# ru1ven/KeypointFusion

Measured on AMD Instinct MI355X. Metric: RGB-D img/sec fwd (B=64, 256x256), higher is better.
Workload: dtype f32; 1 GPU; KPFusion-convnext-tiny, depth+RGB UNet backbones forward, B=64/GPU 256x256 f32 (BASELINE configs[1]); batch_per_gpu=64, global_batch=64, input=256x256, parallelism=dp1 (batch shards, no collective)

## Files before the change

### keypointfusion_amd/csrc/kpf_mlp.hip

```cpp
#include "kpf_common.h"
#include <stdlib.h>
#include <type_traits>

namespace {

typedef __attribute__((address_space(3))) void lds_void_t;
typedef __attribute__((address_space(1))) void gbl_void_t;

__device__ __attribute__((aligned(16))) float kpf_mlp_zero16[4] = {0.f, 0.f, 0.f, 0.f};

struct MlpArgs {
  const float* y;
  const float* x;
  const float* w1;
  const float* b1;
  const float* w2;
  const float* b2;
  const float* gamma;
  float* out;
  const float* zero;
  int M;
};

__device__ __forceinline__ float gelu_f(float x) {
  const float z = fabsf(x) * 0.70710678118654752440f;
  const float t = __builtin_amdgcn_rcpf(fmaf(0.3275911f, z, 1.0f));
  float p = fmaf(1.061405429f, t, -1.453152027f);
  p = fmaf(p, t, 1.421413741f);
  p = fmaf(p, t, -0.284496736f);
  p = fmaf(p, t, 0.254829592f);
  const float e = __builtin_amdgcn_exp2f(-1.4426950408889634f * z * z);
  const float q = 0.5f * x * (p * t) * e;
  return fmaxf(x, 0.f) - fabsf(q);
}

template <int RC>
__device__ __forceinline__ int row_sw(int r) {
  static_assert(RC % 8 == 0, "row length must be a multiple of 32 floats");
  return (RC % 16 == 0) ? (r & 15) : ((r >> 1) & 7);
}

template <int ROWS, int RC, int NT>
__device__ __forceinline__ void dma_image(float* lds_dst, const float* src, long src_ld, int valid_rows, const float* zero, int tid) {
  static_assert((ROWS * RC) % NT == 0, "image must be a whole number of workgroup-wide passes");
  constexpr int PASSES = ROWS * RC / NT;
  const int wave = tid >> 6;
#pragma unroll
  for (int p = 0; p < PASSES; ++p) {
    const int pos = p * NT + tid;
    const int r = pos / RC, cp = pos - r * RC;
    const int c = cp ^ row_sw<RC>(r);
    const float* s = r < valid_rows ? src + (long)r * src_ld + 4 * c : zero;
    __builtin_amdgcn_global_load_lds((gbl_void_t*)s, (lds_void_t*)(lds_dst + (p * NT + wave * 64) * 4), 16, 0, 0);
  }
}

template <int NC, int TM, int HT, int NW>
__global__ __launch_bounds__(64 * NW) void convnext_mlp_kernel(const MlpArgs a) {
  constexpr int NT = 64 * NW;
  constexpr int C = 16 * NC;
  constexpr int H4 = 4 * C;
  constexpr int HC = 16 * HT;
  constexpr int BM = 16 * TM * NW;
  constexpr int RCY = C / 4;
  constexpr int RCW = HC / 4;
  constexpr int NCH = H4 / HC;
  constexpr int YF = BM * C, W1F = HC * C, W2F = C * HC;
  static_assert(H4 % HC == 0, "chunking");

  extern __shared__ __attribute__((aligned(16))) float lds[];
  float* Ys = lds;
  float* W1s = Ys + YF;
  float* W2s = W1s + 2 * W1F;
  float* B1s = W2s + 2 * W2F;

  const int tid = threadIdx.x, lane = tid & 63, wave = tid >> 6;
  const int fr = lane & 15, fg = lane >> 4;
  const long m0 = (long)blockIdx.x * BM;
  const int valid = (int)((a.M - m0) < BM ? (a.M - m0) : BM);

  dma_image<BM, RCY, NT>(Ys, a.y + m0 * C, C, valid, a.zero, tid);
  dma_image<HC, RCY, NT>(W1s, a.w1, C, HC, a.zero, tid);
  dma_image<C, RCW, NT>(W2s, a.w2, H4, C, a.zero, tid);

  const f32x4 zero4 = {0.f, 0.f, 0.f, 0.f};
  f32x4 acc2[NC][TM];
#pragma unroll
  for (int n = 0; n < NC; ++n)
#pragma unroll
    for (int j = 0; j < TM; ++j) acc2[n][j] = zero4;

  float* B2s = B1s + H4;
  float* Gs = B2s + C;
  for (int i = tid; i < H4; i += NT) B1s[i] = a.b1[i];
  for (int i = tid; i < C; i += NT) {
    B2s[i] = a.b2[i];
    Gs[i] = a.gamma[i];
  }
  __syncthreads();

  const int yrow0 = wave * TM * 16 + fr;
  for (int ch = 0; ch < NCH; ++ch) {
    const int cur = ch & 1;
    if (ch + 1 < NCH) {
      dma_image<HC, RCY, NT>(W1s + (cur ^ 1) * W1F, a.w1 + (long)(ch + 1) * HC * C, C, HC, a.zero, tid);
      dma_image<C, RCW, NT>(W2s + (cur ^ 1) * W2F, a.w2 + (long)(ch + 1) * HC, H4, C, a.zero, tid);
    }
    const float* w1b = W1s + cur * W1F;
    const float* w2b = W2s + cur * W2F;

    f32x4 acc1[HT][TM];
#pragma unroll
    for (int h = 0; h < HT; ++h)
#pragma unroll
      for (int j = 0; j < TM; ++j) acc1[h][j] = zero4;
#pragma unroll
    for (int s = 0; s < NC; ++s) {
      f32x4 yf[TM], wf[HT];
#pragma unroll
      for (int j = 0; j < TM; ++j) {
        const int r = yrow0 + j * 16;
        yf[j] = *reinterpret_cast<const f32x4*>(Ys + r * C + (((4 * s + fg) ^ row_sw<RCY>(r)) << 2));
      }
#pragma unroll
      for (int h = 0; h < HT; ++h) {
        const int r = h * 16 + fr;
        wf[h] = *reinterpret_cast<const f32x4*>(w1b + r * C + (((4 * s + fg) ^ row_sw<RCY>(r)) << 2));
      }
#pragma unroll
      for (int e = 0; e < 4; ++e)
#pragma unroll
        for (int h = 0; h < HT; ++h)
#pragma unroll
          for (int j = 0; j < TM; ++j) acc1[h][j] = __builtin_amdgcn_mfma_f32_16x16x4f32(wf[h][e], yf[j][e], acc1[h][j], 0, 0, 0);
    }

#pragma unroll
    for (int h = 0; h < HT; ++h) {
      const f32x4 bv = *reinterpret_cast<const f32x4*>(B1s + ch * HC + h * 16 + 4 * fg);
#pragma unroll
      for (int j = 0; j < TM; ++j)
#pragma unroll
        for (int e = 0; e < 4; ++e) acc1[h][j][e] = gelu_f(acc1[h][j][e] + bv[e]);
      f32x4 wf[NC];
#pragma unroll
      for (int n = 0; n < NC; ++n) {
        const int r = n * 16 + fr;
        wf[n] = *reinterpret_cast<const f32x4*>(w2b + r * HC + (((4 * h + fg) ^ row_sw<RCW>(r)) << 2));
      }
#pragma unroll
      for (int e = 0; e < 4; ++e)
#pragma unroll
        for (int n = 0; n < NC; ++n)
#pragma unroll
          for (int j = 0; j < TM; ++j) acc2[n][j] = __builtin_amdgcn_mfma_f32_16x16x4f32(wf[n][e], acc1[h][j][e], acc2[n][j], 0, 0, 0);
    }
    __syncthreads();
  }

#pragma unroll
  for (int j = 0; j < TM; ++j) {
    const long m = m0 + wave * TM * 16 + j * 16 + fr;
    if (m >= a.M) continue;
    f32x4 xv[NC];
#pragma unroll
    for (int n = 0; n < NC; ++n) xv[n] = *reinterpret_cast<const f32x4*>(a.x + m * C + n * 16 + 4 * fg);
#pragma unroll
    for (int n = 0; n < NC; ++n) {
      const int c = n * 16 + 4 * fg;
      const f32x4 bv = *reinterpret_cast<const f32x4*>(B2s + c);
      const f32x4 gv = *reinterpret_cast<const f32x4*>(Gs + c);
      f32x4 v;
#pragma unroll
      for (int e = 0; e < 4; ++e) v[e] = xv[n][e] + gv[e] * (acc2[n][j][e] + bv[e]);
      *reinterpret_cast<f32x4*>(a.out + m * C + c) = v;
    }
  }
}

struct MlpSplitArgs {
  const float* y;
  const float* x;
  const float* w1;
  const float* b1;
  const float* w2;
  const float* b2;
  const float* gamma;
  float* out;
  const float* zero;
  float us1, us2;
  int M;
};

template <int NC, int HT, int NW, bool YLDS, int TM>
__global__ __launch_bounds__(64 * NW) void convnext_mlp_split_kernel(const MlpSplitArgs a) {
  constexpr int NT = 64 * NW;
  constexpr int C = 16 * NC;
  constexpr int KC = C / 32;
  constexpr int H4 = 4 * C;
  constexpr int HC = 16 * HT;
  constexpr int HK = HC / 32;
  constexpr int BM = 16 * TM * NW;
  constexpr int RCY = C / 4, RCW = HC / 4;
  constexpr int NCH = H4 / HC;
  constexpr int YF = YLDS ? BM * C : 0, W1F = HC * C, W2F = C * HC;
  static_assert(C % 32 == 0 && HC % 32 == 0 && H4 % HC == 0, "split blocks are 32 wide");

  extern __shared__ __attribute__((aligned(16))) float lds[];
  float* Ys = lds;
  float* W1s = Ys + YF;
  float* W2s = W1s + 2 * W1F;
  float* B1s = W2s + 2 * W2F;
  float* B2s = B1s + H4;
  float* Gs = B2s + C;

  const int tid = threadIdx.x, lane = tid & 63, wave = tid >> 6;
  const int fr = lane & 15, fg = lane >> 4;
  const long m0 = (long)blockIdx.x * BM;
  const int valid = (int)((a.M - m0) < BM ? (a.M - m0) : BM);

  if (YLDS) dma_image<BM, RCY, NT>(Ys, a.y + m0 * C, C, valid, a.zero, tid);
  dma_image<HC, RCY, NT>(W1s, a.w1, C, HC, a.zero, tid);
  dma_image<C, RCW, NT>(W2s, a.w2, H4, C, a.zero, tid);

  const f32x4 zero4 = {0.f, 0.f, 0.f, 0.f};
  f32x4 acc2[NC][TM];
#pragma unroll
  for (int n = 0; n < NC; ++n)
#pragma unroll
    for (int j = 0; j < TM; ++j) acc2[n][j] = zero4;
  for (int i = tid; i < H4; i += NT) B1s[i] = a.b1[i];
  for (int i = tid; i < C; i += NT) {
    B2s[i] = a.b2[i];
    Gs[i] = a.gamma[i];
  }
  __syncthreads();

  f16x8 yh[KC][TM], yl[KC][TM];
#pragma unroll
  for (int j = 0; j < TM; ++j) {
    const int yr = (wave * TM + j) * 16 + fr;
    if (YLDS) {
#pragma unroll
      for (int k = 0; k < KC; ++k) {
        yh[k][j] = *reinterpret_cast<const f16x8*>(Ys + yr * C + (((8 * k + fg) ^ row_sw<RCY>(yr)) << 2));
        yl[k][j] = *reinterpret_cast<const f16x8*>(Ys + yr * C + (((8 * k + 4 + fg) ^ row_sw<RCY>(yr)) << 2));
      }
    } else {
      const long mr = (m0 + yr < a.M) ? m0 + yr : a.M - 1;
      const float* yrow = a.y + mr * C;
#pragma unroll
      for (int k = 0; k < KC; ++k) {
        yh[k][j] = *reinterpret_cast<const f16x8*>(yrow + ((8 * k + fg) << 2));
        yl[k][j] = *reinterpret_cast<const f16x8*>(yrow + ((8 * k + 4 + fg) << 2));
      }
    }
  }
  const float us1 = a.us1;

  for (int ch = 0; ch < NCH; ++ch) {
    const int cur = ch & 1;
    if (ch + 1 < NCH) {
      dma_image<HC, RCY, NT>(W1s + (cur ^ 1) * W1F, a.w1 + (long)(ch + 1) * HC * C, C, HC, a.zero, tid);
      dma_image<C, RCW, NT>(W2s + (cur ^ 1) * W2F, a.w2 + (long)(ch + 1) * HC, H4, C, a.zero, tid);
    }
    const float* w1b = W1s + cur * W1F;
    const float* w2b = W2s + cur * W2F;

    f32x4 acc1[HT][TM];
#pragma unroll
    for (int h = 0; h < HT; ++h)
#pragma unroll
      for (int j = 0; j < TM; ++j) acc1[h][j] = zero4;
#pragma unroll
    for (int k = 0; k < KC; ++k) {
#pragma unroll
      for (int h = 0; h < HT; ++h) {
        const int r = h * 16 + fr;
        const f16x8 wh = *reinterpret_cast<const f16x8*>(w1b + r * C + (((8 * k + fg) ^ row_sw<RCY>(r)) << 2));
        const f16x8 wl = *reinterpret_cast<const f16x8*>(w1b + r * C + (((8 * k + 4 + fg) ^ row_sw<RCY>(r)) << 2));
#pragma unroll
        for (int j = 0; j < TM; ++j) {
          acc1[h][j] = __builtin_amdgcn_mfma_f32_16x16x32_f16(wl, yh[k][j], acc1[h][j], 0, 0, 0);
          acc1[h][j] = __builtin_amdgcn_mfma_f32_16x16x32_f16(wh, yl[k][j], acc1[h][j], 0, 0, 0);
          acc1[h][j] = __builtin_amdgcn_mfma_f32_16x16x32_f16(wh, yh[k][j], acc1[h][j], 0, 0, 0);
        }
      }
    }

#pragma unroll
    for (int q = 0; q < HK; ++q) {
      f16x8 hh[TM], hl[TM];
#pragma unroll
      for (int t = 0; t < 2; ++t) {
        const int h = 2 * q + t;
        const f32x4 bv = *reinterpret_cast<const f32x4*>(B1s + ch * HC + h * 16 + 4 * fg);
#pragma unroll
        for (int j = 0; j < TM; ++j)
#pragma unroll
          for (int e = 0; e < 4; ++e) {
            const float g = gelu_f(fmaf(acc1[h][j][e], us1, bv[e]));
            const _Float16 hi = (_Float16)g;
            hh[j][4 * t + e] = hi;
            hl[j][4 * t + e] = (_Float16)(g - (float)hi);
          }
      }
#pragma unroll
      for (int n = 0; n < NC; ++n) {
        const int r = n * 16 + fr;
        const f16x8 wh = *reinterpret_cast<const f16x8*>(w2b + r * HC + (((8 * q + fg) ^ row_sw<RCW>(r)) << 2));
        const f16x8 wl = *reinterpret_cast<const f16x8*>(w2b + r * HC + (((8 * q + 4 + fg) ^ row_sw<RCW>(r)) << 2));
#pragma unroll
        for (int j = 0; j < TM; ++j) {
          acc2[n][j] = __builtin_amdgcn_mfma_f32_16x16x32_f16(wl, hh[j], acc2[n][j], 0, 0, 0);
          acc2[n][j] = __builtin_amdgcn_mfma_f32_16x16x32_f16(wh, hl[j], acc2[n][j], 0, 0, 0);
          acc2[n][j] = __builtin_amdgcn_mfma_f32_16x16x32_f16(wh, hh[j], acc2[n][j], 0, 0, 0);
        }
      }
    }
    __syncthreads();
  }

  const float us2 = a.us2;
#pragma unroll
  for (int j = 0; j < TM; ++j) {
    const long m = m0 + (wave * TM + j) * 16 + fr;
    if (m >= a.M) continue;
    f32x4 xv[NC];
#pragma unroll
    for (int n = 0; n < NC; ++n) xv[n] = *reinterpret_cast<const f32x4*>(a.x + m * C + n * 16 + 4 * fg);
#pragma unroll
    for (int n = 0; n < NC; ++n) {
      const int c = n * 16 + 4 * fg;
      const f32x4 bv = *reinterpret_cast<const f32x4*>(B2s + c);
      const f32x4 gv = *reinterpret_cast<const f32x4*>(Gs + c);
      f32x4 v;
#pragma unroll
      for (int e = 0; e < 4; ++e) v[e] = xv[n][e] + gv[e] * fmaf(acc2[n][j][e], us2, bv[e]);
      *reinterpret_cast<f32x4*>(a.out + m * C + c) = v;
    }
  }
}

struct Mlp16Args {
  const void* y;
  const void* x;
  const void* w1;
  const float* b1;
  const void* w2c;
  const float* b2;
  const float* gamma;
  void* out;
  int M;
  int dbg;
};

__device__ __forceinline__ float gelu_h16m(float x) { return kpf_gelu_h16(x); }

template <int C, int PT, int R, bool BF, int WPS = 2, int NW = 4>
__global__ __launch_bounds__(64 * NW, WPS) void convnext_mlp_h16_kernel(const Mlp16Args a) {
  using TH = typename std::conditional<BF, bf16_t, f16_t>::type;
  constexpr int NT = 64 * NW;
  constexpr int KC = C / 32;
  constexpr int NCT = C / 16;
  constexpr int NCH = 4 * C / 32;
  constexpr int W1B = 32 * C * 2;
  constexpr int W2B = C * 64;
  constexpr int CHB = W1B + W2B;
  constexpr int G = CHB / (NT * 16);
  constexpr int RC1 = C / 8;
  constexpr int BM = 16 * PT * NW;
  static_assert(C % 128 == 0 && R >= 2 && R <= 4 && W1B % (NT * 16) == 0 && W2B % (NT * 16) == 0, "shape");

  extern __shared__ __attribute__((aligned(16))) float lds[];
  char* const LB = reinterpret_cast<char*>(lds);
  constexpr int RING_B = R * CHB > NW * PT * 16 * 2 * C ? R * CHB : NW * PT * 16 * 2 * C;
  float* const B1s = reinterpret_cast<float*>(LB + RING_B);
  float* const B2s = B1s + 4 * C;
  float* const Gs = B2s + C;
  const int tid = threadIdx.x, lane = tid & 63;
  const int wave = __builtin_amdgcn_readfirstlane(tid >> 6);
  const int fr = lane & 15, fg = lane >> 4;
  const long m0 = (long)blockIdx.x * BM;

  f16x8 yf[KC][PT];
#pragma unroll
  for (int pt = 0; pt < PT; ++pt) {
    long m = m0 + (wave * PT + pt) * 16 + fr;
    m = m < a.M ? m : a.M - 1;
    const TH* yrow = reinterpret_cast<const TH*>(a.y) + m * C + 8 * fg;
#pragma unroll
    for (int ks = 0; ks < KC; ++ks) yf[ks][pt] = *reinterpret_cast<const f16x8*>(yrow + 32 * ks);
  }
  for (int i = tid; i < 4 * C; i += NT) B1s[i] = a.b1[i];
  for (int i = tid; i < C; i += NT) {
    B2s[i] = a.b2[i];
    Gs[i] = a.gamma[i];
  }
  __syncthreads();
  asm volatile("s_waitcnt vmcnt(0)" ::: "memory");

  const TH* const w1g = reinterpret_cast<const TH*>(a.w1);
  const TH* const w2g = reinterpret_cast<const TH*>(a.w2c);
  constexpr int P1 = W1B / (NT * 16), P2 = W2B / (NT * 16), RPP1 = NT / RC1;
  const int r1 = tid / RC1, cp1 = tid % RC1;
  const int s1a = r1 * C + 8 * (cp1 ^ (r1 & 15)), s1b = r1 * C + 8 * (cp1 ^ ((r1 + RPP1) & 15));
  const int s2 = (tid >> 2) * 32 + 8 * ((tid & 3) ^ ((tid >> 4) & 3));
  auto stage = [&](int ch, int slot) {
    char* dst = LB + slot * CHB + wave * 1024;
    const TH* const g1 = w1g + (long)ch * 32 * C;
    const TH* const g2 = w2g + (long)ch * C * 32;
#pragma unroll
    for (int p = 0; p < P1; ++p)
      __builtin_amdgcn_global_load_lds((gbl_void_t*)(g1 + ((p & 1) ? s1b : s1a) + p * RPP1 * C), (lds_void_t*)(dst + p * NT * 16), 16, 0, 0);
#pragma unroll
    for (int p = 0; p < P2; ++p)
      __builtin_amdgcn_global_load_lds((gbl_void_t*)(g2 + s2 + p * (NT / 4) * 32), (lds_void_t*)(dst + W1B + p * NT * 16), 16, 0, 0);
  };
  if (!(a.dbg & 4))
#pragma unroll
    for (int c = 0; c < R - 1; ++c) stage(c, c);

  f32x4 acc[NCT][PT];
#pragma unroll
  for (int n = 0; n < NCT; ++n)
#pragma unroll
    for (int pt = 0; pt < PT; ++pt) acc[n][pt] = f32x4{0.f, 0.f, 0.f, 0.f};
  const int w1_rd = fr * (2 * C), w2_rd = W1B + fr * 64 + ((fg ^ ((fr >> 2) & 3)) << 4);

  auto chunk = [&](int ch, auto SLOT) {
    constexpr int slot = decltype(SLOT)::value;
    const int younger = NCH - 1 - ch;
    if (a.dbg & 4) {
    } else if (younger >= R - 2) asm volatile("s_waitcnt vmcnt(%0)" ::"n"((R - 2) * G) : "memory");
    else if (R > 3 && younger == 1) asm volatile("s_waitcnt vmcnt(%0)" ::"n"(G) : "memory");
    else asm volatile("s_waitcnt vmcnt(0)" ::: "memory");
    __builtin_amdgcn_s_barrier();
    if (ch + R - 1 < NCH && !(a.dbg & 4)) stage(ch + R - 1, (slot + R - 1) % R);
    const char* const sb = LB + slot * CHB;
    f32x4 d1[2][PT];
#pragma unroll
    for (int ht = 0; ht < 2; ++ht)
#pragma unroll
      for (int pt = 0; pt < PT; ++pt) d1[ht][pt] = f32x4{0.f, 0.f, 0.f, 0.f};
#pragma unroll
    for (int ks = 0; ks < KC; ++ks)
#pragma unroll
      for (int ht = 0; ht < 2; ++ht) {
        const f16x8 w = *reinterpret_cast<const f16x8*>(sb + w1_rd + ht * 16 * (2 * C) + ((((4 * ks + fg) ^ fr) & (RC1 - 1)) << 4));
#pragma unroll
        for (int pt = 0; pt < PT; ++pt) {
          if constexpr (BF) d1[ht][pt] = __builtin_amdgcn_mfma_f32_16x16x32_bf16(__builtin_bit_cast(bf16x8, w), __builtin_bit_cast(bf16x8, yf[ks][pt]), d1[ht][pt], 0, 0, 0);
          else d1[ht][pt] = __builtin_amdgcn_mfma_f32_16x16x32_f16(w, yf[ks][pt], d1[ht][pt], 0, 0, 0);
        }
      }
    const f32x4 bv0 = *reinterpret_cast<const f32x4*>(B1s + ch * 32 + 4 * fg);
    const f32x4 bv1 = *reinterpret_cast<const f32x4*>(B1s + ch * 32 + 16 + 4 * fg);
    f16x8 hf[PT];
#pragma unroll
    for (int pt = 0; pt < PT; ++pt) {
      typename std::conditional<BF, bf16x8, f16x8>::type h;
#pragma unroll
      for (int e = 0; e < 4; ++e) {
        h[e] = (TH)((a.dbg & 1) ? d1[0][pt][e] + bv0[e] : gelu_h16m(d1[0][pt][e] + bv0[e]));
        h[4 + e] = (TH)((a.dbg & 1) ? d1[1][pt][e] + bv1[e] : gelu_h16m(d1[1][pt][e] + bv1[e]));
      }
      hf[pt] = __builtin_bit_cast(f16x8, h);
    }
#pragma unroll
    for (int n = 0; n < NCT; ++n) {
      const f16x8 w = *reinterpret_cast<const f16x8*>(sb + w2_rd + n * 16 * 64);
#pragma unroll
      for (int pt = 0; pt < PT; ++pt) {
        if constexpr (BF) acc[n][pt] = __builtin_amdgcn_mfma_f32_16x16x32_bf16(__builtin_bit_cast(bf16x8, w), __builtin_bit_cast(bf16x8, hf[pt]), acc[n][pt], 0, 0, 0);
        else acc[n][pt] = __builtin_amdgcn_mfma_f32_16x16x32_f16(w, hf[pt], acc[n][pt], 0, 0, 0);
      }
    }
  };
  static_assert(NCH % R == 0, "whole ring revolutions");
  for (int cb = 0; cb < NCH; cb += R) {
    chunk(cb, std::integral_constant<int, 0>{});
    chunk(cb + 1, std::integral_constant<int, 1 % R>{});
    if constexpr (R > 2) chunk(cb + 2, std::integral_constant<int, 2 % R>{});
    if constexpr (R > 3) chunk(cb + 3, std::integral_constant<int, 3 % R>{});
  }
  __builtin_amdgcn_s_barrier();

  const TH* const xg = reinterpret_cast<const TH*>(a.x);
  TH* const og = reinterpret_cast<TH*>(a.out);
  constexpr int ROWB = 2 * C;
  char* const stg = LB + wave * (PT * 16 * ROWB);
#pragma unroll
  for (int pt = 0; pt < PT; ++pt) {
    const long m = m0 + (wave * PT + pt) * 16 + fr;
    const long mr = m < a.M ? m : a.M - 1;
    f32x4 xv[NCT];
#pragma unroll
    for (int n = 0; n < NCT; ++n) xv[n] = kpf_ld4(xg + mr * C + n * 16 + 4 * fg);
#pragma unroll
    for (int n = 0; n < NCT; ++n) {
      const f32x4 bv = *reinterpret_cast<const f32x4*>(B2s + n * 16 + 4 * fg);
      const f32x4 gv = *reinterpret_cast<const f32x4*>(Gs + n * 16 + 4 * fg);
      f32x4 v;
#pragma unroll
      for (int e = 0; e < 4; ++e) v[e] = xv[n][e] + gv[e] * (acc[n][pt][e] + bv[e]);
      const int row = pt * 16 + fr, cidx = 2 * n + (fg >> 1);
      kpf_st4(reinterpret_cast<TH*>(stg + row * ROWB + ((cidx ^ fr) << 4) + (fg & 1) * 8), v);
    }
  }
  asm volatile("s_waitcnt lgkmcnt(0)" ::: "memory");
  constexpr int CPR = ROWB / 16, RPI = 64 / CPR;
  const int rl = lane / CPR, p = lane % CPR;
#pragma unroll
  for (int it = 0; it < PT * 16 / RPI; ++it) {
    const int row = it * RPI + rl;
    const int c = p ^ (row & 15);
    const f32x4 q = *reinterpret_cast<const f32x4*>(stg + row * ROWB + (p << 4));
    const long m = m0 + wave * PT * 16 + row;
    if (m < a.M && !(a.dbg & 2)) *reinterpret_cast<f32x4*>(og + m * C + 8 * c) = q;
  }
}

template <int C, int PT, int R, int WPS = 2, int NW = 4>
int launch_mlp_h16(const Mlp16Args& a, int dtype, hipStream_t st) {
  constexpr int CHB = 32 * C * 2 + C * 64, BM = 16 * PT * NW;
  constexpr int RING_B = R * CHB > NW * PT * 16 * 2 * C ? R * CHB : NW * PT * 16 * 2 * C;
  const size_t lds = (size_t)RING_B + 6 * C * sizeof(float);
  void (*kern)(const Mlp16Args) = dtype == KPF_DT_BF16 ? convnext_mlp_h16_kernel<C, PT, R, true, WPS, NW> : convnext_mlp_h16_kernel<C, PT, R, false, WPS, NW>;
  static std::atomic<bool> lds_opt_in[2][KPF_MAX_DEVICES];
  if (!kpf_raise_lds_limit(reinterpret_cast<const void*>(kern), lds_opt_in[dtype == KPF_DT_BF16 ? 1 : 0])) {
    kpf_set_error("kpf_convnext_mlp_h16: cannot raise the dynamic LDS limit");
    return KPF_ELAUNCH;
  }
  const long tiles = ((long)a.M + BM - 1) / BM;
  hipLaunchKernelGGL(kern, dim3((unsigned)tiles), dim3(64 * NW), lds, st, a);
  return kpf_check_launch("kpf_convnext_mlp_h16");
}

template <int NC, int HT, int NW, bool YLDS, int TM>
int launch_mlp_split(MlpSplitArgs& a, hipStream_t st) {
  constexpr int C = 16 * NC, HC = 16 * HT, BM = 16 * TM * NW;
  const size_t lds = (size_t)((YLDS ? BM * C : 0) + 2 * HC * C + 2 * C * HC + 6 * C) * sizeof(float);
  auto kern = convnext_mlp_split_kernel<NC, HT, NW, YLDS, TM>;
  static std::atomic<bool> lds_opt_in[KPF_MAX_DEVICES];
  if (!kpf_raise_lds_limit(reinterpret_cast<const void*>(kern), lds_opt_in)) {
    kpf_set_error("kpf_convnext_mlp_split_f32: cannot raise the dynamic LDS limit");
    return KPF_ELAUNCH;
  }
  const long tiles = (a.M + BM - 1) / BM;
  hipLaunchKernelGGL(kern, dim3((unsigned)tiles), dim3(64 * NW), lds, st, a);
  return kpf_check_launch("kpf_convnext_mlp_split_f32");
}

template <int NC, int TM, int HT, int NW>
int launch_mlp(MlpArgs& a, hipStream_t st) {
  constexpr int C = 16 * NC, HC = 16 * HT, BM = 16 * TM * NW;
  const size_t lds = (size_t)(BM * C + 2 * HC * C + 2 * C * HC + 6 * C) * sizeof(float);
  auto kern = convnext_mlp_kernel<NC, TM, HT, NW>;
  static std::atomic<bool> lds_opt_in[KPF_MAX_DEVICES];
  if (!kpf_raise_lds_limit(reinterpret_cast<const void*>(kern), lds_opt_in)) {
    kpf_set_error("kpf_convnext_mlp_f32: cannot raise the dynamic LDS limit");
    return KPF_ELAUNCH;
  }
  const long tiles = (a.M + BM - 1) / BM;
  hipLaunchKernelGGL(kern, dim3((unsigned)tiles), dim3(64 * NW), lds, st, a);
  return kpf_check_launch("kpf_convnext_mlp_f32");
}

}

extern "C" int kpf_convnext_mlp_supported(int C) { return C == 96 || C == 128; }

extern "C" int kpf_convnext_mlp_f32(const float* y, const float* x, const float* w1, const float* b1, const float* w2, const float* b2,
                                    const float* gamma, float* out, long M, int C, void* stream) {
  KPF_REQUIRE(y && x && w1 && b1 && w2 && b2 && gamma && out && M > 0, "kpf_convnext_mlp_f32: null pointer / empty");
  KPF_REQUIRE(C == 96 || C == 128 || C == 192, "kpf_convnext_mlp_f32: C=%d not supported (96, 128, 192)", C);
  KPF_REQUIRE(M < (1l << 31), "kpf_convnext_mlp_f32: too many rows");
  KPF_REQUIRE(kpf_aligned16(y) && kpf_aligned16(x) && kpf_aligned16(w1) && kpf_aligned16(w2) && kpf_aligned16(out) && kpf_aligned16(b1) &&
                  kpf_aligned16(b2) && kpf_aligned16(gamma),
              "kpf_convnext_mlp_f32: pointers must be 16-byte aligned");
  MlpArgs a;
  a.y = y; a.x = x; a.w1 = w1; a.b1 = b1; a.w2 = w2; a.b2 = b2; a.gamma = gamma; a.out = out; a.M = (int)M;
  {
    static const float* zero_of_dev[64] = {nullptr};
    int dev = 0;
    if (hipGetDevice(&dev) != hipSuccess || dev < 0 || dev >= 64) dev = 0;
    if (!zero_of_dev[dev]) {
      void* p = nullptr;
      if (hipGetSymbolAddress(&p, HIP_SYMBOL(kpf_mlp_zero16)) != hipSuccess || !p) {
        kpf_set_error("kpf_convnext_mlp_f32: cannot resolve the zero page");
        return KPF_ELAUNCH;
      }
      zero_of_dev[dev] = static_cast<const float*>(p);
    }
    a.zero = zero_of_dev[dev];
  }
  hipStream_t st = reinterpret_cast<hipStream_t>(stream);
  switch (C) {
    case 96: return launch_mlp<6, 1, 4, 8>(a, st);
    case 128: return launch_mlp<8, 1, 2, 8>(a, st);
    default: return launch_mlp<12, 1, 2, 4>(a, st);
  }
}

static const float* mlp_zero_page() {
  static const float* zero_of_dev[64] = {nullptr};
  int dev = 0;
  if (hipGetDevice(&dev) != hipSuccess || dev < 0 || dev >= 64) dev = 0;
  if (!zero_of_dev[dev]) {
    void* p = nullptr;
    if (hipGetSymbolAddress(&p, HIP_SYMBOL(kpf_mlp_zero16)) != hipSuccess || !p) return nullptr;
    zero_of_dev[dev] = static_cast<const float*>(p);
  }
  return zero_of_dev[dev];
}

extern "C" int kpf_convnext_mlp_h16_supported(int C) { return C == 128 || C == 256; }

extern "C" int kpf_convnext_mlp_h16(const void* y, const void* x, const void* w1, const float* b1, const void* w2_chunks, const float* b2,
                                    const float* gamma, void* out, long M, int C, int dtype, void* stream) {
  KPF_REQUIRE(y && x && w1 && b1 && w2_chunks && b2 && gamma && out && M > 0, "kpf_convnext_mlp_h16: null pointer / empty");
  KPF_REQUIRE(kpf_convnext_mlp_h16_supported(C), "kpf_convnext_mlp_h16: C=%d not supported (128, 256)", C);
  KPF_REQUIRE(dtype == KPF_DT_BF16 || dtype == KPF_DT_F16, "kpf_convnext_mlp_h16: dtype must be KPF_DT_BF16 or KPF_DT_F16");
  KPF_REQUIRE(M < (1l << 31), "kpf_convnext_mlp_h16: too many rows");
  KPF_REQUIRE(kpf_aligned16(y) && kpf_aligned16(x) && kpf_aligned16(w1) && kpf_aligned16(w2_chunks) && kpf_aligned16(out) && kpf_aligned16(b1) &&
                  kpf_aligned16(b2) && kpf_aligned16(gamma),
              "kpf_convnext_mlp_h16: pointers must be 16-byte aligned");
  Mlp16Args a;
  a.y = y; a.x = x; a.w1 = w1; a.b1 = b1; a.w2c = w2_chunks; a.b2 = b2; a.gamma = gamma; a.out = out; a.M = (int)M;
  static const int dbg = []() { const char* e = getenv("KPF_MLP16_DBG"); return e ? atoi(e) : 0; }();
  a.dbg = dbg;
  hipStream_t st = reinterpret_cast<hipStream_t>(stream);
  static const int cfg = []() { const char* e = getenv("KPF_MLP16_CFG"); return e ? atoi(e) : 0; }();
  if (C == 128 && cfg == 5) return launch_mlp_h16<128, 3, 4, 2, 8>(a, dtype, st);
  if (C == 128) return launch_mlp_h16<128, 3, 4>(a, dtype, st);
  return launch_mlp_h16<256, 2, 2>(a, dtype, st);
}

extern "C" int kpf_convnext_mlp_split_supported(int C) { return C == 96 || C == 128 || C == 192 || C == 256; }

extern "C" int kpf_convnext_mlp_split_f32(const float* y_split, const float* x, const float* w1_split, const float* b1, float w1_unscale,
                                          const float* w2_split_perm, const float* b2, float w2_unscale, const float* gamma, float* out, long M,
                                          int C, void* stream) {
  KPF_REQUIRE(y_split && x && w1_split && b1 && w2_split_perm && b2 && gamma && out && M > 0, "kpf_convnext_mlp_split_f32: null pointer / empty");
  KPF_REQUIRE(kpf_convnext_mlp_split_supported(C), "kpf_convnext_mlp_split_f32: C=%d not supported (96, 128, 192, 256)", C);
  KPF_REQUIRE(M < (1l << 31) && w1_unscale > 0.f && w2_unscale > 0.f, "kpf_convnext_mlp_split_f32: bad M / scales");
  KPF_REQUIRE(kpf_aligned16(y_split) && kpf_aligned16(x) && kpf_aligned16(w1_split) && kpf_aligned16(w2_split_perm) && kpf_aligned16(out) &&
                  kpf_aligned16(b1) && kpf_aligned16(b2) && kpf_aligned16(gamma),
              "kpf_convnext_mlp_split_f32: pointers must be 16-byte aligned");
  MlpSplitArgs a;
  a.y = y_split; a.x = x; a.w1 = w1_split; a.b1 = b1; a.w2 = w2_split_perm; a.b2 = b2; a.gamma = gamma; a.out = out; a.M = (int)M;
  a.us1 = w1_unscale; a.us2 = w2_unscale;
  a.zero = mlp_zero_page();
  KPF_REQUIRE(a.zero, "kpf_convnext_mlp_split_f32: cannot resolve the zero page");
  hipStream_t st = reinterpret_cast<hipStream_t>(stream);
  static const int tm_env = []() { const char* e = getenv("KPF_MLP_TM"); return e ? atoi(e) : 2; }();
  if (tm_env == 1) {
    if (C == 96) return launch_mlp_split<6, 4, 8, true, 1>(a, st);
    if (C == 128) return launch_mlp_split<8, 2, 8, true, 1>(a, st);
    if (C == 192) return launch_mlp_split<12, 2, 8, false, 1>(a, st);
    return launch_mlp_split<16, 2, 8, false, 1>(a, st);
  }
  if (C == 96) return launch_mlp_split<6, 4, 8, false, 2>(a, st);
  if (C == 128) return launch_mlp_split<8, 2, 8, false, 2>(a, st);
  if (C == 192) return launch_mlp_split<12, 2, 8, false, 2>(a, st);
  return launch_mlp_split<16, 2, 8, false, 1>(a, st);
}
```

Measured before the change: 3499 img/s.

## Keep MLP activation tile in registers and prefetch residual for C=96/128

Adds a ConvNeXt MLP kernel variant that loads each wave's input rows straight into registers instead of staging the whole Y tile in LDS. Dropping the Y tile shrinks LDS use so more workgroups can fit per CU. The residual input x is loaded before the last hidden chunk so its latency overlaps with compute. Tile shape changes (TM=2, 4 waves, 2 waves-per-EU hint), which raises register pressure and may cause spills; optional cycle-stamp instrumentation and an env switch back to the old kernel are also included.

```diff
diff --git a/keypointfusion_amd/csrc/kpf_mlp.hip b/keypointfusion_amd/csrc/kpf_mlp.hip
--- a/keypointfusion_amd/csrc/kpf_mlp.hip
+++ b/keypointfusion_amd/csrc/kpf_mlp.hip
@@ -55,6 +55,15 @@
   }
 }
 
+#ifdef KPF_DBG_TIME
+__device__ unsigned long long kpf_mlp_dbg_t[8 * 8192];
+#define MLP_STAMP(i) do { if (threadIdx.x == 0 && blockIdx.x < 8192) { kpf_mlp_dbg_t[8 * blockIdx.x + (i)] = __builtin_readcyclecounter(); \
+    if ((i) == 0) { kpf_mlp_dbg_t[8 * blockIdx.x + 4] = __builtin_amdgcn_s_memrealtime(); kpf_mlp_dbg_t[8 * blockIdx.x + 6] = __builtin_amdgcn_s_getreg((4 << 0) | (0 << 6) | (31 << 11)) | ((unsigned long long)__builtin_amdgcn_s_getreg((20 << 0) | (0 << 6) | (3 << 11)) << 32); } \
+    if ((i) == 3) kpf_mlp_dbg_t[8 * blockIdx.x + 5] = __builtin_amdgcn_s_memrealtime(); } } while (0)
+#else
+#define MLP_STAMP(i) do { } while (0)
+#endif
+
 template <int NC, int TM, int HT, int NW>
 __global__ __launch_bounds__(64 * NW) void convnext_mlp_kernel(const MlpArgs a) {
   constexpr int NT = 64 * NW;
@@ -78,6 +87,7 @@
   const int fr = lane & 15, fg = lane >> 4;
   const long m0 = (long)blockIdx.x * BM;
   const int valid = (int)((a.M - m0) < BM ? (a.M - m0) : BM);
+  MLP_STAMP(0);
 
   dma_image<BM, RCY, NT>(Ys, a.y + m0 * C, C, valid, a.zero, tid);
   dma_image<HC, RCY, NT>(W1s, a.w1, C, HC, a.zero, tid);
@@ -98,6 +108,7 @@
     Gs[i] = a.gamma[i];
   }
   __syncthreads();
+  MLP_STAMP(1);
 
   const int yrow0 = wave * TM * 16 + fr;
   for (int ch = 0; ch < NCH; ++ch) {
@@ -157,6 +168,7 @@
     }
     __syncthreads();
   }
+  MLP_STAMP(2);
 
 #pragma unroll
   for (int j = 0; j < TM; ++j) {
@@ -176,6 +188,136 @@
       *reinterpret_cast<f32x4*>(a.out + m * C + c) = v;
     }
   }
+  MLP_STAMP(3);
+}
+
+template <int NC, int TM, int HT, int NW, int WPS>
+__global__ __launch_bounds__(64 * NW, WPS) void convnext_mlp_reg_kernel(const MlpArgs a) {
+  constexpr int NT = 64 * NW;
+  constexpr int C = 16 * NC, H4 = 4 * C, HC = 16 * HT;
+  constexpr int BM = 16 * TM * NW;
+  constexpr int RCY = C / 4, RCW = HC / 4;
+  constexpr int NCH = H4 / HC;
+  constexpr int W1F = HC * C, W2F = C * HC;
+  static_assert(H4 % HC == 0 && NCH >= 2, "chunking");
+
+  extern __shared__ __attribute__((aligned(16))) float lds[];
+  float* W1s = lds;
+  float* W2s = W1s + 2 * W1F;
+  float* B1s = W2s + 2 * W2F;
+  float* B2s = B1s + H4;
+  float* Gs = B2s + C;
+
+  const int tid = threadIdx.x, lane = tid & 63, wave = tid >> 6;
+  const int fr = lane & 15, fg = lane >> 4;
+  const long m0 = (long)blockIdx.x * BM;
+  MLP_STAMP(0);
+
+  long mrow[TM];
+  f32x4 yf[NC][TM];
+#pragma unroll
+  for (int j = 0; j < TM; ++j) {
+    const long m = m0 + (wave * TM + j) * 16 + fr;
+    mrow[j] = m < a.M ? m : (long)a.M - 1;
+    const float* yrow = a.y + mrow[j] * C + 4 * fg;
+#pragma unroll
+    for (int s = 0; s < NC; ++s) yf[s][j] = *reinterpret_cast<const f32x4*>(yrow + 16 * s);
+  }
+  dma_image<HC, RCY, NT>(W1s, a.w1, C, HC, a.zero, tid);
+  dma_image<C, RCW, NT>(W2s, a.w2, H4, C, a.zero, tid);
+
+  const f32x4 zero4 = {0.f, 0.f, 0.f, 0.f};
+  f32x4 acc2[NC][TM];
+#pragma unroll
+  for (int n = 0; n < NC; ++n)
+#pragma unroll
+    for (int j = 0; j < TM; ++j) acc2[n][j] = zero4;
+  for (int i = tid; i < H4; i += NT) B1s[i] = a.b1[i];
+  for (int i = tid; i < C; i += NT) {
+    B2s[i] = a.b2[i];
+    Gs[i] = a.gamma[i];
+  }
+  __syncthreads();
+  MLP_STAMP(1);
+
+  auto chunk = [&](const int ch) __attribute__((always_inline)) {
+    const int cur = ch & 1;
+    if (ch + 1 < NCH) {
+      dma_image<HC, RCY, NT>(W1s + (cur ^ 1) * W1F, a.w1 + (long)(ch + 1) * HC * C, C, HC, a.zero, tid);
+      dma_image<C, RCW, NT>(W2s + (cur ^ 1) * W2F, a.w2 + (long)(ch + 1) * HC, H4, C, a.zero, tid);
+    }
+    const float* w1b = W1s + cur * W1F;
+    const float* w2b = W2s + cur * W2F;
+
+    f32x4 acc1[HT][TM];
+#pragma unroll
+    for (int h = 0; h < HT; ++h)
+#pragma unroll
+      for (int j = 0; j < TM; ++j) acc1[h][j] = zero4;
+#pragma unroll
+    for (int s = 0; s < NC; ++s) {
+      f32x4 wf[HT];
+#pragma unroll
+      for (int h = 0; h < HT; ++h) {
+        const int r = h * 16 + fr;
+        wf[h] = *reinterpret_cast<const f32x4*>(w1b + r * C + (((4 * s + fg) ^ row_sw<RCY>(r)) << 2));
+      }
+#pragma unroll
+      for (int e = 0; e < 4; ++e)
+#pragma unroll
+        for (int h = 0; h < HT; ++h)
+#pragma unroll
+          for (int j = 0; j < TM; ++j) acc1[h][j] = __builtin_amdgcn_mfma_f32_16x16x4f32(wf[h][e], yf[s][j][e], acc1[h][j], 0, 0, 0);
+    }
+
+#pragma unroll
+    for (int h = 0; h < HT; ++h) {
+      const f32x4 bv = *reinterpret_cast<const f32x4*>(B1s + ch * HC + h * 16 + 4 * fg);
+#pragma unroll
+      for (int j = 0; j < TM; ++j)
+#pragma unroll
+        for (int e = 0; e < 4; ++e) acc1[h][j][e] = gelu_f(acc1[h][j][e] + bv[e]);
+      f32x4 wf[NC];
+#pragma unroll
+      for (int n = 0; n < NC; ++n) {
+        const int r = n * 16 + fr;
+        wf[n] = *reinterpret_cast<const f32x4*>(w2b + r * HC + (((4 * h + fg) ^ row_sw<RCW>(r)) << 2));
+      }
+#pragma unroll
+      for (int e = 0; e < 4; ++e)
+#pragma unroll
+        for (int n = 0; n < NC; ++n)
+#pragma unroll
+          for (int j = 0; j < TM; ++j) acc2[n][j] = __builtin_amdgcn_mfma_f32_16x16x4f32(wf[n][e], acc1[h][j][e], acc2[n][j], 0, 0, 0);
+    }
+    __syncthreads();
+  };
+
+  for (int ch = 0; ch < NCH - 1; ++ch) chunk(ch);
+  f32x4 xv[NC][TM];
+#pragma unroll
+  for (int j = 0; j < TM; ++j)
+#pragma unroll
+    for (int n = 0; n < NC; ++n) xv[n][j] = *reinterpret_cast<const f32x4*>(a.x + mrow[j] * C + n * 16 + 4 * fg);
+  chunk(NCH - 1);
+  MLP_STAMP(2);
+
+#pragma unroll
+  for (int j = 0; j < TM; ++j) {
+    const long m = m0 + (wave * TM + j) * 16 + fr;
+    if (m >= a.M) continue;
+#pragma unroll
+    for (int n = 0; n < NC; ++n) {
+      const int c = n * 16 + 4 * fg;
+      const f32x4 bv = *reinterpret_cast<const f32x4*>(B2s + c);
+      const f32x4 gv = *reinterpret_cast<const f32x4*>(Gs + c);
+      f32x4 v;
+#pragma unroll
+      for (int e = 0; e < 4; ++e) v[e] = xv[n][j][e] + gv[e] * (acc2[n][j][e] + bv[e]);
+      *reinterpret_cast<f32x4*>(a.out + m * C + c) = v;
+    }
+  }
+  MLP_STAMP(3);
 }
 
 struct MlpSplitArgs {
@@ -557,6 +699,21 @@
   constexpr int C = 16 * NC, HC = 16 * HT, BM = 16 * TM * NW;
   const size_t lds = (size_t)(BM * C + 2 * HC * C + 2 * C * HC + 6 * C) * sizeof(float);
   auto kern = convnext_mlp_kernel<NC, TM, HT, NW>;
+  static std::atomic<bool> lds_opt_in[KPF_MAX_DEVICES];
+  if (!kpf_raise_lds_limit(reinterpret_cast<const void*>(kern), lds_opt_in)) {
+    kpf_set_error("kpf_convnext_mlp_f32: cannot raise the dynamic LDS limit");
+    return KPF_ELAUNCH;
+  }
+  const long tiles = (a.M + BM - 1) / BM;
+  hipLaunchKernelGGL(kern, dim3((unsigned)tiles), dim3(64 * NW), lds, st, a);
+  return kpf_check_launch("kpf_convnext_mlp_f32");
+}
+
+template <int NC, int TM, int HT, int NW, int WPS>
+int launch_mlp_reg(MlpArgs& a, hipStream_t st) {
+  constexpr int C = 16 * NC, HC = 16 * HT, BM = 16 * TM * NW;
+  const size_t lds = (size_t)(2 * HC * C + 2 * C * HC + 6 * C) * sizeof(float);
+  auto kern = convnext_mlp_reg_kernel<NC, TM, HT, NW, WPS>;
   static std::atomic<bool> lds_opt_in[KPF_MAX_DEVICES];
   if (!kpf_raise_lds_limit(reinterpret_cast<const void*>(kern), lds_opt_in)) {
     kpf_set_error("kpf_convnext_mlp_f32: cannot raise the dynamic LDS limit");
@@ -596,9 +753,15 @@
     a.zero = zero_of_dev[dev];
   }
   hipStream_t st = reinterpret_cast<hipStream_t>(stream);
+  const char* fe = getenv("KPF_MLP_FORM");
+  const int form = fe ? atoi(fe) : 0;
   switch (C) {
-    case 96: return launch_mlp<6, 1, 4, 8>(a, st);
-    case 128: return launch_mlp<8, 1, 2, 8>(a, st);
+    case 96:
+      if (form == 1) return launch_mlp<6, 1, 4, 8>(a, st);
+      return launch_mlp_reg<6, 2, 2, 4, 2>(a, st);
+    case 128:
+      if (form == 1) return launch_mlp<8, 1, 2, 8>(a, st);
+      return launch_mlp_reg<8, 2, 2, 4, 2>(a, st);
     default: return launch_mlp<12, 1, 2, 4>(a, st);
   }
 }
@@ -614,6 +777,16 @@
   }
   return zero_of_dev[dev];
 }
+
+#ifdef KPF_DBG_TIME
+extern "C" int kpf_mlp_dbg_read(unsigned long long* host, int n) {
+  return hipMemcpyFromSymbol(host, HIP_SYMBOL(kpf_mlp_dbg_t), sizeof(unsigned long long) * n) == hipSuccess ? 0 : -1;
+}
+extern "C" int kpf_mlp_dbg_clear(void) {
+  static unsigned long long z[8 * 8192] = {0};
+  return hipMemcpyToSymbol(HIP_SYMBOL(kpf_mlp_dbg_t), z, sizeof(z)) == hipSuccess ? 0 : -1;
+}
+#endif
 
 extern "C" int kpf_convnext_mlp_h16_supported(int C) { return C == 128 || C == 256; }
 
```

Measured after the change: 3527 img/s (median of 6 runs). No clear change (+0.8%).

## Add persistent ConvNeXt MLP kernel that streams weights across row tiles

Applied to the files above, without the earlier changes.

Adds a persistent-grid variant of the fused ConvNeXt MLP kernel, launched with one workgroup per CU, which loops over row tiles. It keeps the Y tile in registers instead of LDS and prefetches the next tile's first weight chunk and input rows during the last chunk of the current tile. The aim is to cut per-tile launch and prologue cost and to overlap weight DMA with compute. The C=128 case also moves to a larger hidden chunk. Each block now re-streams all weights for every tile, and LDS-free Y loads may raise register pressure. Optional cycle-stamp instrumentation is compiled in only under a debug macro.

```diff
diff --git a/keypointfusion_amd/csrc/kpf_mlp.hip b/keypointfusion_amd/csrc/kpf_mlp.hip
--- a/keypointfusion_amd/csrc/kpf_mlp.hip
+++ b/keypointfusion_amd/csrc/kpf_mlp.hip
@@ -55,6 +55,15 @@
   }
 }
 
+#ifdef KPF_DBG_TIME
+__device__ unsigned long long kpf_mlp_dbg_t[8 * 8192];
+#define KPF_MLP_STAMP(tile, i) do { if (threadIdx.x == 0 && (tile) < 8192) { kpf_mlp_dbg_t[8 * (tile) + (i)] = __builtin_readcyclecounter(); \
+    if ((i) == 0) kpf_mlp_dbg_t[8 * (tile) + 4] = __builtin_amdgcn_s_memrealtime(); \
+    if ((i) == 3) kpf_mlp_dbg_t[8 * (tile) + 5] = __builtin_amdgcn_s_memrealtime(); } } while (0)
+#else
+#define KPF_MLP_STAMP(tile, i)
+#endif
+
 template <int NC, int TM, int HT, int NW>
 __global__ __launch_bounds__(64 * NW) void convnext_mlp_kernel(const MlpArgs a) {
   constexpr int NT = 64 * NW;
@@ -78,6 +87,7 @@
   const int fr = lane & 15, fg = lane >> 4;
   const long m0 = (long)blockIdx.x * BM;
   const int valid = (int)((a.M - m0) < BM ? (a.M - m0) : BM);
+  KPF_MLP_STAMP(blockIdx.x, 0);
 
   dma_image<BM, RCY, NT>(Ys, a.y + m0 * C, C, valid, a.zero, tid);
   dma_image<HC, RCY, NT>(W1s, a.w1, C, HC, a.zero, tid);
@@ -100,6 +110,7 @@
   __syncthreads();
 
   const int yrow0 = wave * TM * 16 + fr;
+  KPF_MLP_STAMP(blockIdx.x, 1);
   for (int ch = 0; ch < NCH; ++ch) {
     const int cur = ch & 1;
     if (ch + 1 < NCH) {
@@ -158,6 +169,7 @@
     __syncthreads();
   }
 
+  KPF_MLP_STAMP(blockIdx.x, 2);
 #pragma unroll
   for (int j = 0; j < TM; ++j) {
     const long m = m0 + wave * TM * 16 + j * 16 + fr;
@@ -175,6 +187,151 @@
       for (int e = 0; e < 4; ++e) v[e] = xv[n][e] + gv[e] * (acc2[n][j][e] + bv[e]);
       *reinterpret_cast<f32x4*>(a.out + m * C + c) = v;
     }
+  }
+  KPF_MLP_STAMP(blockIdx.x, 3);
+}
+
+
+template <int NC, int TM, int HT, int NW, int WPE>
+__global__ __launch_bounds__(64 * NW, WPE) void convnext_mlp_persistent_kernel(const MlpArgs a, const int tiles) {
+  constexpr int NT = 64 * NW;
+  constexpr int C = 16 * NC, H4 = 4 * C, HC = 16 * HT;
+  constexpr int BM = 16 * TM * NW;
+  constexpr int RCY = C / 4, RCW = HC / 4;
+  constexpr int NCH = H4 / HC;
+  constexpr int W1F = HC * C, W2F = C * HC;
+  static_assert(H4 % HC == 0 && NCH % 2 == 0, "an even number of chunks keeps chunk c in buffer c & 1 across tiles");
+
+  extern __shared__ __attribute__((aligned(16))) float lds[];
+  float* W1s = lds;
+  float* W2s = W1s + 2 * W1F;
+  float* B1s = W2s + 2 * W2F;
+  float* B2s = B1s + H4;
+  float* Gs = B2s + C;
+
+  const int tid = threadIdx.x, lane = tid & 63, wave = tid >> 6;
+  const int fr = lane & 15, fg = lane >> 4;
+  const int row0 = wave * TM * 16 + fr;
+  const long M = a.M;
+
+  for (int i = tid; i < H4; i += NT) B1s[i] = a.b1[i];
+  for (int i = tid; i < C; i += NT) {
+    B2s[i] = a.b2[i];
+    Gs[i] = a.gamma[i];
+  }
+  dma_image<HC, RCY, NT>(W1s, a.w1, C, HC, a.zero, tid);
+  dma_image<C, RCW, NT>(W2s, a.w2, H4, C, a.zero, tid);
+
+  f32x4 yf[NC][TM];
+  auto load_y = [&](long tile) {
+#pragma unroll
+    for (int j = 0; j < TM; ++j) {
+      long m = tile * BM + row0 + j * 16;
+      m = m < M ? m : M - 1;
+      const float* yr = a.y + m * C + 4 * fg;
+#pragma unroll
+      for (int s = 0; s < NC; ++s) yf[s][j] = *reinterpret_cast<const f32x4*>(yr + 16 * s);
+    }
+  };
+  load_y(blockIdx.x);
+  __syncthreads();
+
+  const f32x4 zero4 = {0.f, 0.f, 0.f, 0.f};
+  for (long tile = blockIdx.x; tile < tiles; tile += gridDim.x) {
+    KPF_MLP_STAMP(tile, 0);
+    const bool more = tile + gridDim.x < tiles;
+    f32x4 acc2[NC][TM], xv[TM][NC];
+#pragma unroll
+    for (int n = 0; n < NC; ++n)
+#pragma unroll
+      for (int j = 0; j < TM; ++j) acc2[n][j] = zero4;
+
+    auto chunk = [&](const int ch, auto LAST) {
+      constexpr bool last = decltype(LAST)::value;
+      const int cur = ch & 1;
+      if (!last || more) {
+        const int nx = last ? 0 : ch + 1;
+        dma_image<HC, RCY, NT>(W1s + (cur ^ 1) * W1F, a.w1 + (long)nx * HC * C, C, HC, a.zero, tid);
+        dma_image<C, RCW, NT>(W2s + (cur ^ 1) * W2F, a.w2 + (long)nx * HC, H4, C, a.zero, tid);
+      }
+      if constexpr (last) {
+#pragma unroll
+        for (int j = 0; j < TM; ++j) {
+          long m = tile * BM + row0 + j * 16;
+          m = m < M ? m : M - 1;
+#pragma unroll
+          for (int n = 0; n < NC; ++n) xv[j][n] = *reinterpret_cast<const f32x4*>(a.x + m * C + n * 16 + 4 * fg);
+        }
+      }
+      const float* w1b = W1s + cur * W1F;
+      const float* w2b = W2s + cur * W2F;
+
+      f32x4 acc1[HT][TM];
+#pragma unroll
+      for (int h = 0; h < HT; ++h)
+#pragma unroll
+        for (int j = 0; j < TM; ++j) acc1[h][j] = zero4;
+#pragma unroll
+      for (int s = 0; s < NC; ++s) {
+        f32x4 wf[HT];
+#pragma unroll
+        for (int h = 0; h < HT; ++h) {
+          const int r = h * 16 + fr;
+          wf[h] = *reinterpret_cast<const f32x4*>(w1b + r * C + (((4 * s + fg) ^ row_sw<RCY>(r)) << 2));
+        }
+#pragma unroll
+        for (int e = 0; e < 4; ++e)
+#pragma unroll
+          for (int h = 0; h < HT; ++h)
+#pragma unroll
+            for (int j = 0; j < TM; ++j) acc1[h][j] = __builtin_amdgcn_mfma_f32_16x16x4f32(wf[h][e], yf[s][j][e], acc1[h][j], 0, 0, 0);
+      }
+      if constexpr (last)
+        if (more) load_y(tile + gridDim.x);
+
+#pragma unroll
+      for (int h = 0; h < HT; ++h) {
+        const f32x4 bv = *reinterpret_cast<const f32x4*>(B1s + ch * HC + h * 16 + 4 * fg);
+#pragma unroll
+        for (int j = 0; j < TM; ++j)
+#pragma unroll
+          for (int e = 0; e < 4; ++e) acc1[h][j][e] = gelu_f(acc1[h][j][e] + bv[e]);
+        f32x4 wf[NC];
+#pragma unroll
+        for (int n = 0; n < NC; ++n) {
+          const int r = n * 16 + fr;
+          wf[n] = *reinterpret_cast<const f32x4*>(w2b + r * HC + (((4 * h + fg) ^ row_sw<RCW>(r)) << 2));
+        }
+#pragma unroll
+        for (int e = 0; e < 4; ++e)
+#pragma unroll
+          for (int n = 0; n < NC; ++n)
+#pragma unroll
+            for (int j = 0; j < TM; ++j) acc2[n][j] = __builtin_amdgcn_mfma_f32_16x16x4f32(wf[n][e], acc1[h][j][e], acc2[n][j], 0, 0, 0);
+      }
+      __syncthreads();
+    };
+    KPF_MLP_STAMP(tile, 1);
+    for (int ch = 0; ch < NCH - 1; ++ch) chunk(ch, std::false_type{});
+    chunk(NCH - 1, std::true_type{});
+    KPF_MLP_STAMP(tile, 2);
+
+#pragma unroll
+    for (int j = 0; j < TM; ++j) {
+      const long m = tile * BM + row0 + j * 16;
+      if (m >= M) continue;
+#pragma unroll
+      for (int n = 0; n < NC; ++n) {
+        const int c = n * 16 + 4 * fg;
+        const f32x4 bv = *reinterpret_cast<const f32x4*>(B2s + c);
+        const f32x4 gv = *reinterpret_cast<const f32x4*>(Gs + c);
+        f32x4 v;
+#pragma unroll
+        for (int e = 0; e < 4; ++e) v[e] = xv[j][n][e] + gv[e] * (acc2[n][j][e] + bv[e]);
+        *reinterpret_cast<f32x4*>(a.out + m * C + c) = v;
+      }
+    }
+    KPF_MLP_STAMP(tile, 3);
   }
 }
 
@@ -567,7 +724,50 @@
   return kpf_check_launch("kpf_convnext_mlp_f32");
 }
 
-}
+int mlp_cu_count() {
+  static std::atomic<int> cus[KPF_MAX_DEVICES];
+  int dev = 0;
+  if (hipGetDevice(&dev) != hipSuccess || dev < 0 || dev >= KPF_MAX_DEVICES) return 0;
+  int n = cus[dev].load(std::memory_order_acquire);
+  if (n > 0) return n;
+  if (hipDeviceGetAttribute(&n, hipDeviceAttributeMultiprocessorCount, dev) != hipSuccess || n <= 0) return 0;
+  cus[dev].store(n, std::memory_order_release);
+  return n;
+}
+
+template <int NC, int TM, int HT, int NW, int WPC>
+int launch_mlp_persistent(MlpArgs& a, hipStream_t st) {
+  constexpr int C = 16 * NC, HC = 16 * HT, BM = 16 * TM * NW;
+  constexpr int WPE = NW * WPC / 4;
+  constexpr size_t lds = (size_t)(2 * HC * C + 2 * C * HC + 6 * C) * sizeof(float);
+  static_assert(WPC * lds <= 160 * 1024 && WPE >= 1 && WPE <= 8, "workgroups per CU");
+  auto kern = convnext_mlp_persistent_kernel<NC, TM, HT, NW, WPE>;
+  static std::atomic<bool> lds_opt_in[KPF_MAX_DEVICES];
+  if (!kpf_raise_lds_limit(reinterpret_cast<const void*>(kern), lds_opt_in)) {
+    kpf_set_error("kpf_convnext_mlp_f32: cannot raise the dynamic LDS limit");
+    return KPF_ELAUNCH;
+  }
+  const int cus = mlp_cu_count();
+  if (cus <= 0) {
+    kpf_set_error("kpf_convnext_mlp_f32: cannot read the CU count");
+    return KPF_ELAUNCH;
+  }
+  const long tiles = (a.M + BM - 1) / BM, slots = (long)cus * WPC;
+  hipLaunchKernelGGL(kern, dim3((unsigned)(tiles < slots ? tiles : slots)), dim3(64 * NW), lds, st, a, (int)tiles);
+  return kpf_check_launch("kpf_convnext_mlp_f32");
+}
+
+}
+
+#ifdef KPF_DBG_TIME
+extern "C" int kpf_mlp_dbg_read(unsigned long long* host, int n) {
+  return hipMemcpyFromSymbol(host, HIP_SYMBOL(kpf_mlp_dbg_t), sizeof(unsigned long long) * n) == hipSuccess ? 0 : -1;
+}
+extern "C" int kpf_mlp_dbg_clear(void) {
+  static unsigned long long z[8 * 8192];
+  return hipMemcpyToSymbol(HIP_SYMBOL(kpf_mlp_dbg_t), z, sizeof(z)) == hipSuccess ? 0 : -1;
+}
+#endif
 
 extern "C" int kpf_convnext_mlp_supported(int C) { return C == 96 || C == 128; }
 
@@ -596,6 +796,13 @@
     a.zero = zero_of_dev[dev];
   }
   hipStream_t st = reinterpret_cast<hipStream_t>(stream);
+  const char* v1 = getenv("KPF_MLP_V1");
+  if (!(v1 && atoi(v1) != 0) && C != 192) {
+    if (C == 96) return launch_mlp_persistent<6, 1, 4, 8, 1>(a, st);
+    const char* ce = getenv("KPF_MLP_CFG");
+    if (ce && atoi(ce) == 1) return launch_mlp_persistent<8, 1, 2, 8, 1>(a, st);
+    return launch_mlp_persistent<8, 1, 4, 8, 1>(a, st);
+  }
   switch (C) {
     case 96: return launch_mlp<6, 1, 4, 8>(a, st);
     case 128: return launch_mlp<8, 1, 2, 8>(a, st);
```

Measured after the change: 3502 img/s before, 3538 img/s after (median of 6 runs). +1.1%, better.
